# yardenas/ethz-safe-learning

Measured on AMD Instinct MI355X. Metric: planning steps/sec (CEM-MPC, N=2000 K=5 H=30), higher is better.
Workload: dtype f32

## Files before the change

ethz_safe_learning_amd/_capi.py:

```python
from __future__ import annotations

import ctypes as C
import os

CEM_ABI_VERSION = 4
CEM_MAX_ACT = 32
CEM_MAX_COST_KINDS = 4
CEM_COMM_ID_BYTES = 128
CEM_MAX_BATCH = 256
CEM_TRAIN_MAX_BATCH = 4096
CEM_INIT_COLD, CEM_INIT_EXPLICIT, CEM_INIT_SHIFT = 0, 1, 2
CEM_VARIANT_CEM, CEM_VARIANT_SAFE, CEM_VARIANT_COST = 0, 1, 2
CEM_PARTICLES_MEAN, CEM_PARTICLES_LOWER_TAIL = 0, 1
CEM_CONSTRAINT_BETA, CEM_CONSTRAINT_BUDGET = 0, 1
CEM_REFIT_UNIFORM, CEM_REFIT_SOFTMAX = 0, 1
CEM_NOISE_WHITE, CEM_NOISE_MIXED = 0, 1
CEM_FORWARD_SPLIT, CEM_FORWARD_ALL = 0, 1

_HERE = os.path.dirname(os.path.abspath(__file__))
LIB_PATH = os.environ.get('CEM_MPC_LIB') or os.path.join(_HERE, 'lib', 'libcem_mpc_gfx950.so')

EXPORTED_SYMBOLS = [
    'cem_abi_version', 'cem_status_string', 'cem_last_hip_error', 'cem_weight_blob_floats',
    'cem_packed_weight_floats', 'cem_workspace_bytes', 'cem_pack_weights_host', 'cem_plan_tiles_host', 'cem_plan_segments_host', 'cem_rollout_residency',
    'cem_planner_create', 'cem_planner_destroy', 'cem_planner_layout', 'cem_planner_set_weights', 'cem_planner_set_weights_dev',
    'cem_planner_set_normaliser', 'cem_planner_plan', 'cem_plan_begin', 'cem_plan_rollout', 'cem_plan_select',
    'cem_plan_end', 'cem_comm_unique_id', 'cem_planner_comm_init', 'cem_planner_comm_destroy', 'cem_planner_comm_ranks', 'cem_plan_exchange', 'cem_planner_graph_status', 'cem_planner_launches_per_iteration', 'cem_planner_rollout_path', 'cem_unfold_sequences', 'cem_compute_objective', 'cem_scorer_reward', 'cem_scorer_cost', 'cem_fill_noise', 'cem_philox_words', 'cem_planner_set_timing', 'cem_planner_last_timing', 'cem_planner_last_timing_detail', 'cem_planner_select_mode', 'cem_planner_inject_fault',
    'cem_batch_workspace_bytes', 'cem_batch_planner_create', 'cem_planner_plan_batch', 'cem_planner_batch_capacity',
    'cem_planner_set_warm_start', 'cem_planner_set_initial_distribution', 'cem_planner_set_init_mode', 'cem_planner_reset_carry',
    'cem_planner_get_carry', 'cem_planner_set_carry_slots', 'cem_planner_set_particle_objective', 'cem_planner_get_particle_objective',
    'cem_planner_set_constraint', 'cem_planner_get_constraint', 'cem_planner_set_cost_budget', 'cem_planner_constraint_costs',
    'cem_planner_set_refit', 'cem_planner_get_refit', 'cem_planner_refit_stats',
    'cem_planner_set_action_noise', 'cem_planner_get_action_noise', 'cem_planner_action_noise_dev',
    'cem_trainer_workspace_bytes', 'cem_trainer_blob_floats', 'cem_trainer_create', 'cem_trainer_destroy', 'cem_trainer_set_state',
    'cem_trainer_get_state', 'cem_trainer_weights_dev', 'cem_trainer_step', 'cem_trainer_steps', 'cem_trainer_eval', 'cem_trainer_forward',
]


class CemScorer(C.Structure):
    _fields_ = [
        ('goal_mode', C.c_int32), ('goal_lo', C.c_int32), ('goal_hi', C.c_int32),
        ('lidar_max_dist', C.c_float), ('goal_size', C.c_float), ('goal_reached_dist', C.c_float), ('reward_distance', C.c_float),
        ('reward_goal', C.c_float), ('reward_clip', C.c_float),
        ('constrain_indicator', C.c_int32), ('n_cost_kinds', C.c_int32),
        ('cost_lo', C.c_int32 * CEM_MAX_COST_KINDS), ('cost_hi', C.c_int32 * CEM_MAX_COST_KINDS),
        ('cost_size', C.c_float * CEM_MAX_COST_KINDS),
    ]


class CemConfig(C.Structure):
# ... 69 lines not shown
    lib.cem_planner_set_weights.argtypes = [vp, vp, C.c_size_t]
    lib.cem_planner_set_weights_dev.argtypes = [vp, vp, C.c_size_t]
    lib.cem_planner_set_normaliser.argtypes = [vp, vp, vp]
    lib.cem_planner_plan.argtypes = [vp, vp, C.c_uint64, C.c_uint64, vp, vp, vp, vp, fp, i32p]
    lib.cem_plan_begin.argtypes = [vp, vp, C.c_uint64, C.c_uint64, vp, vp]
    lib.cem_plan_rollout.argtypes = [vp, C.c_int32]
    lib.cem_plan_select.argtypes = [vp, C.c_int32]
    lib.cem_plan_end.argtypes = [vp, vp, vp, fp, i32p]
    lib.cem_unfold_sequences.argtypes = [vp, vp, vp, C.c_int32, C.c_int32, vp, C.c_uint64, C.c_uint64, vp, vp, vp]
    lib.cem_comm_unique_id.argtypes = [vp]
    lib.cem_planner_comm_init.argtypes = [vp, vp, C.c_int32, C.c_int32]
    lib.cem_planner_comm_destroy.argtypes = [vp]
    lib.cem_plan_exchange.argtypes = [vp]
    lib.cem_planner_graph_status.argtypes = [vp, i32p]
    lib.cem_planner_comm_ranks.argtypes = [vp, i32p]
    lib.cem_planner_launches_per_iteration.argtypes = [vp, i32p]
    lib.cem_planner_rollout_path.argtypes = [vp, i32p]
    lib.cem_compute_objective.argtypes = [vp, vp, C.c_int32, C.c_int32, vp]
    lib.cem_scorer_reward.argtypes = [vp, vp, vp, C.c_int32, vp, vp]
    lib.cem_scorer_cost.argtypes = [vp, vp, C.c_int32, vp]
    lib.cem_fill_noise.argtypes = [vp, C.c_uint64, C.c_uint64, vp, vp, vp]
    lib.cem_philox_words.argtypes = [vp, C.c_uint64, C.c_uint64] + [C.c_uint32] * 6 + [vp]
    lib.cem_planner_select_mode.argtypes = [vp, i32p]
    lib.cem_planner_inject_fault.argtypes = [vp, C.c_int32]
    lib.cem_planner_set_timing.argtypes = [vp, C.c_int32]
    lib.cem_planner_last_timing.argtypes = [vp, fp, i32p, fp]
    lib.cem_planner_last_timing_detail.argtypes = [vp, fp, fp]
    lib.cem_batch_workspace_bytes.restype = C.c_size_t
    lib.cem_batch_workspace_bytes.argtypes = [cfgp, C.c_int32]
    lib.cem_batch_planner_create.argtypes = [cfgp, C.c_int32, vp, C.c_size_t, vp, C.POINTER(vp)]
    lib.cem_planner_plan_batch.argtypes = [vp, C.c_int32, vp, C.c_uint64, vp, vp, vp, vp, vp, vp, vp]
    lib.cem_planner_batch_capacity.argtypes = [vp, i32p]
    lib.cem_planner_set_warm_start.argtypes = [vp, C.POINTER(CemWarmStart)]
    lib.cem_planner_set_initial_distribution.argtypes = [vp, C.c_int32, vp, vp]
    lib.cem_planner_set_init_mode.argtypes = [vp, C.c_int32, C.c_int32]
    lib.cem_planner_reset_carry.argtypes = [vp, C.c_int32]
    lib.cem_planner_get_carry.argtypes = [vp, C.c_int32, vp, vp, i32p]
    lib.cem_planner_set_carry_slots.argtypes = [vp, C.c_int32, vp]
    lib.cem_planner_set_particle_objective.argtypes = [vp, C.c_int32, C.c_int32]
    lib.cem_planner_get_particle_objective.argtypes = [vp, i32p, i32p]
    lib.cem_planner_set_constraint.argtypes = [vp, C.c_int32, C.c_int32]
    lib.cem_planner_get_constraint.argtypes = [vp, i32p, i32p]
    lib.cem_planner_set_cost_budget.argtypes = [vp, vp, C.c_int32]
    lib.cem_planner_constraint_costs.argtypes = [vp, C.c_int32, vp, C.c_int32]
    lib.cem_planner_set_refit.argtypes = [vp, C.c_int32, C.c_float]
    lib.cem_planner_get_refit.argtypes = [vp, i32p, fp]
# ... 32 lines not shown
```

ethz_safe_learning_amd/csrc/cem_capi.hip:

```cpp
#include "cem_device.h"
#include "cem_rollout_lean.h"
#include "cem_score.h"
#include "cem_refit_weighted.h"
#include "cem_noise_mix.h"
#include "cem_train.h"
#include "cem_train_tile.h"
#include "cem_forward.h"
#include "cem_rollout_split.h"
#include "cem_rollout_wide.h"
#include "cem_pack.h"
#include "../../include/cem_mpc.h"

#include <dlfcn.h>
#include <link.h>

#include <algorithm>
#include <atomic>
#include <chrono>
#include <cmath>
#include <cstdio>
#include <cstdlib>
#include <cstring>
#include <limits>
#include <mutex>
#include <new>
#include <string>
#include <type_traits>
// ... 6 lines not shown

struct Dims {
    int O, A, Din, U, L, E, P, N, H, k, I, W, R;
    int Nloc, n_off, Bloc, Btot;
    int KB_in, KB_obs, NFW, KF0;
    int act_q0, act_nq;
    bool wide;
    bool split;
    int wave_groups[4]; uint32_t wave_off_f4[4]; uint32_t member_stride_f4;
    size_t nat_member_floats;
};

int resolve_select_mode(int requested, long long N, long long k, long long HA, size_t dyn_limit, bool can_fuse, bool *cache_out)
{
    const size_t base = (size_t)((k + 3) & ~3ll) * 4 + (size_t)2 * HA * 4;
    const bool one_wg_ok = k <= 24576 && base <= dyn_limit;
    const bool cache = one_wg_ok && base + (size_t)CEM_SEL_KWORDS(N) * 4 <= dyn_limit;
    if (cache_out) *cache_out = cache;
    int mode = requested;
    if (mode == 0) mode = (N >= 24000 || !cache) ? 3 : 1;
    if (mode == 1 && !one_wg_ok) return 0;
    if (mode == 3 && !can_fuse) mode = 2;
    return mode;
}

int validate(const cem_config_t *c)
{
    if (!c) return CEM_ERR_INVALID_ARG;
    if (c->abi_version != CEM_ABI_VERSION) return CEM_ERR_INVALID_ARG;
    if (c->obs_dim < 1 || c->act_dim < 1 || c->act_dim > CEM_MAX_ACT || c->n_layers < 1 || c->ensemble_size < 1 ||
        c->particles < 1 || c->n_samples < 1 || c->horizon < 1 || c->horizon > 65535 || c->iterations < 1 || c->iterations > 65535 ||
        c->n_elite < 1 || c->n_elite > c->n_samples || c->world_size < 1 || c->rank < 0 || c->rank >= c->world_size)
        return CEM_ERR_INVALID_ARG;
    if (c->units < 1) return CEM_ERR_INVALID_ARG;
    if (c->activation < CEM_ACT_RELU || c->activation > CEM_ACT_GELU) return CEM_ERR_INVALID_ARG;
    if (!(fabs((double)c->one_minus_smoothing - (1.0 - (double)c->smoothing)) <= 2e-7)) return CEM_ERR_INVALID_ARG;
    if (c->units > CEM_WIDE_U) return CEM_ERR_UNSUPPORTED;
    if (c->obs_dim + c->act_dim > CEM_U) return CEM_ERR_UNSUPPORTED;
    if (c->n_samples % c->world_size != 0) return CEM_ERR_INVALID_ARG;
    if (((long long)c->particles * c->n_samples) % c->ensemble_size != 0) return CEM_ERR_SPLIT;
    if (c->select_mode >= 0 && c->select_mode <= 3 &&
        resolve_select_mode(c->select_mode, c->n_samples, c->n_elite, (long long)c->horizon * c->act_dim, 140 * 1024, true, nullptr) == 0)
        return CEM_ERR_UNSUPPORTED;
    if (c->scorer.n_cost_kinds < 0 || c->scorer.n_cost_kinds > CEM_MAX_COST_KINDS) return CEM_ERR_INVALID_ARG;
    {
        const cem_scorer_t &s = c->scorer;
// ... 507 lines not shown
        dl_iterate_phdr(count_hip_runtimes, &libs);
        if (libs.size() > 1) {
            std::fprintf(stderr, "cem_mpc: %zu HIP runtimes are loaded in this process:", libs.size());
            for (const auto &l : libs) std::fprintf(stderr, " %s", l.c_str());
            std::fprintf(stderr, "\ncem_mpc: device memory and streams of one are foreign to the other — load libcem_mpc_gfx950.so AFTER the runtime that owns them (INTEGRATION.md)\n");
        }
    });
}
}

struct cem_planner {
    cem_config_t cfg;
    Dims d;
    Layout lay;
    char *ws;
    hipStream_t stream;
    bool own_stream;
    int rc;
    int n_tiles;
    int n_seg, seg_len, n_pinned;
    bool have_weights;
    bool in_plan;
    bool sample_in_rollout;
    bool lean_rollout;
    const float *eps_act, *eps_model;
    CtrlBlock *h_ctrl;
    float *h_result;
    WarmCtl *h_warm; const WarmCtl *d_h_warm;
    uint32_t plan_seq;
    const CtrlBlock *d_h_ctrl; float *d_h_result;
    bool timing; std::vector<hipEvent_t> ev; float roll_ms, sel_ms, red_ms, samp_ms; int roll_n;
    std::vector<std::pair<int, int>> ev_kind;
    hipGraph_t graph; hipGraphExec_t gexec; bool graph_ready;
    ScorerDev sc;
    ScorerDev sc_roll;
    float alpha, beta;
    void *comm;
    int plans_since_comm;
    bool graph_failed;
    size_t sel_dyn_limit;
    int fused_resident;
    bool sel_zeroed;
    bool fuse_banned;
    bool inject_capture_fail;
    uint32_t inject_next;
    char *scratch; size_t scratch_bytes;
// ... 172 lines not shown
{
    int st = mb ? validate_batch(cfg, mb) : validate(cfg); if (st) return st;
    if (!workspace || !out) return CEM_ERR_INVALID_ARG;
    warn_if_two_hip_runtimes();
    cem_planner *h = new (std::nothrow) cem_planner();
    if (!h) return CEM_ERR_INVALID_ARG;
    h->cfg = *cfg; h->d = make_dims(cfg);
    h->batch = mb; h->n_states = warm_slots(h);
    const size_t nb = (size_t)warm_slots(h);
    h->lay = make_layout(cfg, h->d, max_tiles_of(h->d), mb);
    if (workspace_bytes < h->lay.total || ((uintptr_t)workspace & 255)) { delete h; return CEM_ERR_WORKSPACE; }
    h->ws = (char *)workspace; h->stream = (hipStream_t)hip_stream; h->own_stream = false;
    if (!h->stream) {
        if (hipStreamCreateWithFlags(&h->stream, hipStreamNonBlocking) != hipSuccess) { g_last_hip = (int)hipGetLastError(); delete h; return CEM_ERR_HIP; }
        h->own_stream = true;
    }
    { const Plan pl = make_plan(cfg, h->d, mb); h->rc = pl.rc; h->n_seg = pl.n_seg; h->seg_len = pl.seg_len; h->n_pinned = pl.n_pinned;
      const int slots = real_cus() * ((h->d.wide || h->d.split) ? 1 : resident_workgroups(h->d.NFW, pl.rc, pl.n_seg > 1));
      h->sample_in_rollout = (long long)nb * pl.n_tiles <= slots;
      if (const char *e = std::getenv("CEM_FORCE_SAMPLER"))
          h->sample_in_rollout = std::strcmp(e, "kernel") != 0;
      h->lean_rollout = lean_eligible(h, pl.rc);
      if (const char *e = std::getenv("CEM_FORCE_ROLLOUT"))
          h->lean_rollout = h->lean_rollout && std::strcmp(e, "generic") != 0; }
    h->have_weights = false; h->in_plan = false; h->eps_act = h->eps_model = nullptr;
    h->timing = false; h->roll_ms = h->sel_ms = h->red_ms = h->samp_ms = 0.f; h->roll_n = 0;
    h->graph = nullptr; h->gexec = nullptr; h->graph_ready = false; h->tail_m = 0;
    h->cost_m = 0; h->budget_dev = nullptr; h->cstat_obj = nullptr; h->cstat_obj_n = 0; h->last_cstat = nullptr; h->last_cstat_n = h->last_cstat_problems = 0;
    h->refit_kind = CEM_REFIT_UNIFORM; h->refit_tau = 0.f; h->refit_beta = 0.f; h->refit_dev = nullptr; h->refit_ran = false;
    h->noise_kind = CEM_NOISE_WHITE; h->noise_dev = nullptr; h->noise_eps = nullptr; h->noise_floats = 0;
    h->h_budget.assign(nb, std::numeric_limits<float>::infinity());
    h->comm = nullptr; h->plans_since_comm = 0; h->graph_failed = false;
    h->h_ctrl = nullptr; h->h_result = nullptr; h->h_warm = nullptr; h->d_h_warm = nullptr; h->pack_desc = nullptr; h->n_pack_desc = 0;
    h->warm = cem_warm_start_t{}; h->warm.shift = 1; h->warm_staged = 0; h->warm_save_skipped = false;
    h->slot_mode.assign(nb, CEM_INIT_COLD); h->carry_valid.assign(nb, 0); h->have_expl.assign(nb, 0); h->carry_at.assign(nb, -1);
    h->slot_of.resize(nb); for (size_t b = 0; b < nb; ++b) h->slot_of[b] = (int32_t)b;
    h->h_expl.assign(nb * 2 * h->d.H * h->d.A, 0.f);
    h->scratch = nullptr; h->scratch_bytes = 0; h->sel_zeroed = false; h->plan_seq = 0; h->fuse_banned = false; h->inject_next = 0; h->inject_capture_fail = false;
    auto fail = [&](int status) { g_last_hip = (int)hipGetLastError(); release_handle(h); return status; };
    const size_t result_bytes = mb ? nb * CEM_RESULT_WORDS * 4 : 64 * 4;
    if (hipHostMalloc((void **)&h->h_ctrl, nb * sizeof(CtrlBlock), hipHostMallocMapped | hipHostMallocCoherent) != hipSuccess ||
        hipHostMalloc((void **)&h->h_result, result_bytes, hipHostMallocMapped | hipHostMallocCoherent) != hipSuccess ||
        hipHostMalloc((void **)&h->h_warm, sizeof(WarmCtl) + nb * sizeof(WarmProb), hipHostMallocMapped | hipHostMallocCoherent) != hipSuccess) return fail(CEM_ERR_HIP);
    {
        const std::vector<PackDesc> table = build_pack_table(h->d);
        h->n_pack_desc = (uint32_t)table.size();
        const size_t image_bytes = h->d.wide ? wide_image_floats(h->d) * 4 : (size_t)h->d.member_stride_f4 * 16 - 4096;
// ... 482 lines not shown
        if (!h->sel_zeroed) HIPCHK(hipMemsetAsync(m.hist, 0, CEM_MS_CLEAR_BYTES, h->stream));
        h->sel_zeroed = false;
        if (mode == 3) {
            hipLaunchKernelGGL(cem_msel_fused_kernel, dim3(m.G), dim3(1024), 0, h->stream, m);
            hipLaunchKernelGGL(cem_msel_solo_kernel, dim3(1), dim3(1024), 0, h->stream, m);
        } else {
            hipLaunchKernelGGL(cem_msel_hist_kernel<0>, dim3(m.G), dim3(1024), 0, h->stream, m);
            hipLaunchKernelGGL(cem_msel_hist_kernel<1>, dim3(m.G), dim3(1024), 0, h->stream, m);
            hipLaunchKernelGGL(cem_msel_hist_kernel<2>, dim3(m.G), dim3(1024), 0, h->stream, m);
            hipLaunchKernelGGL(cem_msel_count_kernel, dim3(m.G), dim3(1024), 0, h->stream, m);
            hipLaunchKernelGGL(cem_msel_compact_kernel, dim3(m.G), dim3(1024), 0, h->stream, m);
            hipLaunchKernelGGL(cem_msel_moments_kernel<0>, dim3(m.G2), dim3(256), 0, h->stream, m);
            hipLaunchKernelGGL(cem_msel_moments_kernel<1>, dim3(m.G2), dim3(256), 0, h->stream, m);
            hipLaunchKernelGGL(cem_msel_final_kernel, dim3(1), dim3(256), 0, h->stream, m);
        }
    } else {
        if (fold_final && !h->batch && !weighted) {
            p.is_last = it == d.I - 1;
            p.result = h->d_h_result; p.result_dev = (uint32_t *)(ws + l.result); p.eps_out = have_eps_out ? (const float *)(ws + l.eps_out) : nullptr; p.noise_stddev = h->cfg.noise_stddev;
            if (folded) *folded = true;
        }
        if (cache) lds += (size_t)CEM_SEL_KWORDS(d.N) * 4;
        const dim3 grid(warm_slots(h));
        if (cache && h->cfg.variant != CEM_VARIANT_CEM) hipLaunchKernelGGL((cem_select_kernel<true, true>), grid, dim3(1024), lds, h->stream, p);
        else if (cache) hipLaunchKernelGGL((cem_select_kernel<true, false>), grid, dim3(1024), lds, h->stream, p);
        else hipLaunchKernelGGL((cem_select_kernel<false, false>), grid, dim3(1024), lds, h->stream, p);
        if (weighted) {
            HIPCHK(hipGetLastError());
            RefitWeightedParams rw{}; rw.scores = p.scores; rw.actions = p.actions; rw.musig = (float *)(ws + l.musig); rw.ctrl = p.ctrl; rw.elite_idx = p.elite_idx;
            rw.stat = h->refit_dev + (size_t)warm_slots(h) * 2 * p.HA;
            rw.N = d.N; rw.k = d.k; rw.HA = p.HA; rw.I = d.I; rw.beta = h->refit_beta;
            rw.smoothing = p.smoothing; rw.one_minus_smoothing = p.one_minus_smoothing; rw.threshold = h->cfg.stddev_threshold;
            HIPCHK(launch_refit_weighted(rw, warm_slots(h), h->stream));
            h->refit_ran = true;
        }
    }
    HIPCHK(hipGetLastError());
    return CEM_OK;
}

int enqueue_exchange(cem_planner *h)
{
    if (!h->comm) return CEM_OK;
    Rccl *r = rccl(); if (!r) return CEM_ERR_COMM;
    const Dims &d = h->d; const Layout &l = h->lay;
    NCCLCHK(r->AllGather(h->ws + l.scores_local, h->ws + l.scores_global, (size_t)d.Nloc, kNcclFloat32, h->comm, h->stream));
    return CEM_OK;
// ... 778 lines not shown
    HIPCHK(hipStreamSynchronize(h->stream));
    return CEM_OK;
}

int cem_philox_words(cem_planner_t *h, uint64_t seed, uint64_t call, uint32_t stream, uint32_t iteration, uint32_t t, uint32_t sub,
                     uint32_t idx0, uint32_t n, uint32_t *words_out_dev)
{
    if (!h || !words_out_dev || stream > 2 || iteration > 65535 || t > 65535 || sub > 65535) return CEM_ERR_INVALID_ARG;
    if (h->in_plan) return CEM_ERR_STATE;
    if (n == 0) return CEM_OK;
    int st = upload_key(h, seed, call); if (st) return st;
    WordsParams wp{}; wp.out = words_out_dev; wp.ctrl = (const CtrlBlock *)(h->ws + h->lay.ctrl);
    wp.stream = stream; wp.it = iteration; wp.t = t; wp.sub = sub; wp.idx0 = idx0; wp.n = n;
    hipLaunchKernelGGL(cem_philox_words_kernel, dim3((n + 255) / 256), dim3(256), 0, h->stream, wp);
    HIPCHK(hipGetLastError());
    HIPCHK(hipStreamSynchronize(h->stream));
    return CEM_OK;
}

int cem_planner_select_mode(const cem_planner_t *h, int32_t *mode_out)
{
    if (!h || !mode_out) return CEM_ERR_INVALID_ARG;
    *mode_out = select_mode_now(h);
    return CEM_OK;
}

int cem_planner_inject_fault(cem_planner_t *h, int32_t kind)
{
    if (!h || (kind != 1 && kind != 2)) return CEM_ERR_INVALID_ARG;
    if (h->in_plan) return CEM_ERR_STATE;
    if (kind == 2) { h->inject_capture_fail = true; return CEM_OK; }
    h->inject_next = 1u;
    return CEM_OK;
}

int cem_planner_set_timing(cem_planner_t *h, int32_t enable)
{
    if (!h) return CEM_ERR_INVALID_ARG;
    h->timing = enable != 0;
    return CEM_OK;
}

int cem_planner_last_timing(cem_planner_t *h, float *rollout_ms_total, int32_t *rollout_launches, float *select_ms_total)
{
    if (!h) return CEM_ERR_INVALID_ARG;
    if (rollout_ms_total) *rollout_ms_total = h->roll_ms;
// ... 303 lines not shown
```

ethz_safe_learning_amd/csrc/cem_device.h:

```cpp
#pragma once
#include <hip/hip_runtime.h>
#include <stdint.h>

typedef float f4 __attribute__((ext_vector_type(4)));

#define CEM_U 128
#define CEM_ET_NMIN 0
#define CEM_ET_RDELTA 1
#define CEM_ET_BMU 2
#define CEM_ET_BVAR 3
#define CEM_ET_OBS 4
#define CEM_ET_ACT 5
#define CEM_ET_SEL0 6
#define CEM_ET_SEL1 7
#define CEM_ET_ROWS 8
#define CEM_NG 8
#define CEM_NKIND 5
#define CEM_PART_FLOATS (CEM_NKIND * 4 * 64)
#define CEM_TAB_LDS_BYTES (CEM_ET_ROWS * CEM_U * 4)
#define CEM_ROLLOUT_LDS_BYTES(RC_) ((size_t)2 * (RC_) * CEM_NG * 1024 + CEM_PART_FLOATS * 4 + CEM_TAB_LDS_BYTES)

struct TileDesc {
    int32_t row_base;
    int32_t cnt;
// ... 893 lines not shown

struct ScorerOpParams {
    const float *obs, *next_obs; float *out; uint8_t *flag;
    int32_t n, O, what;
    ScorerDev sc;
};

__global__ __launch_bounds__(256) void cem_scorer_kernel(const ScorerOpParams p)
{
    const int row = (int)((blockIdx.x * 256u + threadIdx.x) >> 4), j = threadIdx.x & 15;
    if (row >= p.n) return;
    const float *o = p.obs + (size_t)row * p.O;
    if (p.what == 1) {
        const float c = cem_cost16(o, p.sc, j);
        if (j == 0) p.out[row] = c;
        return;
    }
    const float d = cem_goal_dist16(o, p.sc, j), dn = cem_goal_dist16(p.next_obs + (size_t)row * p.O, p.sc, j);
    const bool ga = d <= p.sc.goal_thresh;
    const float r = cem_reward_of(d, dn, ga, p.sc);
    if (j == 0) { p.out[row] = r; if (p.flag) p.flag[row] = ga ? 1 : 0; }
}

__device__ __forceinline__ float cem_out_noise(const CtrlBlock *ctrl, const float *eps_out, const int a)
{
    if (eps_out) return eps_out[a];
    const f4 e = cem_normal4((uint32_t)(a >> 2), 0u, 0u, 0u, CEM_STREAM_OUT, cem_key(ctrl));
    return e[a & 3];
}


#define CEM_RESULT_WORDS 38
#define CEM_RESULT_MAGIC 0x5EC0DE5Au
__host__ __device__ inline uint32_t cem_result_checksum(const volatile uint32_t *w, const uint32_t seq)
{
    uint32_t x = CEM_RESULT_MAGIC ^ seq;
    for (int i = 0; i < 36; ++i) x = (x ^ w[i]) * 0x01000193u;
    return x ^ (x >> 15);
}
__device__ __forceinline__ void cem_emit_result(float *result, uint32_t *result_dev, const uint32_t *res_l , const uint32_t seq, const int lane)
{
    const uint32_t x = cem_result_checksum(res_l, seq);
    if (lane < CEM_RESULT_WORDS) {
        const uint32_t w = lane < 36 ? res_l[lane] : (lane == 36 ? seq : x);
        if (result_dev) result_dev[lane] = w;
        __hip_atomic_store(reinterpret_cast<uint32_t *>(result) + lane, w, __ATOMIC_RELAXED, __HIP_MEMORY_SCOPE_SYSTEM);
// ... 69 lines not shown
    const int b0 = 2 * tid, b1 = 2 * tid + 1;
    uint32_t h0 = 0u, h1 = 0u;
    if (COHERENT) {
        if (b0 < nbins) h0 = __hip_atomic_load(h + b0, __ATOMIC_RELAXED, __HIP_MEMORY_SCOPE_AGENT);
        if (b1 < nbins) h1 = __hip_atomic_load(h + b1, __ATOMIC_RELAXED, __HIP_MEMORY_SCOPE_AGENT);
    } else { h0 = b0 < nbins ? h[b0] : 0u; h1 = b1 < nbins ? h[b1] : 0u; }
    const uint32_t tot = h0 + h1;
    uint32_t inc = tot;
#pragma unroll
    for (int d = 1; d < 64; d <<= 1) { const uint32_t o = __shfl_up(inc, d); if (lane >= d) inc += o; }
    if (lane == 63) sh[wv] = inc;
    __syncthreads();
    uint32_t before = 0, all = 0;
    for (int i = 0; i < 16; ++i) { const uint32_t v = sh[i]; all += v; if (i < wv) before += v; }
    const uint32_t above = all - (before + inc);
    const uint32_t ge1 = h1 + above, ge0 = tot + above;
    if (ge1 >= need && above < need) { sh[16] = (uint32_t)b1; sh[17] = need - above; }
    if (ge0 >= need && ge1 < need) { sh[16] = (uint32_t)b0; sh[17] = need - ge1; }
    __syncthreads();
    bin = sh[16]; need_next = sh[17];
    __syncthreads();
}

template <bool CACHE, bool CROWDED = false>
__global__ __launch_bounds__(1024) void cem_select_kernel(const SelectParams p)
{
    extern __shared__ __attribute__((aligned(16))) char sel_smem[];
    __shared__ __attribute__((aligned(16))) uint32_t hist[2][256];
    __shared__ uint32_t wsum[2][16];
    __shared__ uint32_t sh_prefix, sh_need, sh_cnt;
    __shared__ uint32_t sh20[20];
    __shared__ __attribute__((aligned(16))) float red[4096];
    __shared__ float bsc[16];
    __shared__ int bpos[16];
    const int prob = (int)blockIdx.x;
    CtrlBlock *const ctrl = p.ctrl + prob;
    if (p.check_done && ctrl->done) return;
    const float *const scores_b = p.scores + (size_t)prob * p.N;
    const float *const actions_b = p.actions + (size_t)prob * p.N * p.HA;
    float *const musig_b = p.musig + (size_t)prob * 2 * p.HA;
    int32_t *const elite_b = p.elite_idx + (size_t)prob * p.k;
    const float *const ret_b = p.ret ? p.ret + (size_t)prob * p.P * p.N : p.ret;
    float *const scores_wb = p.scores_w ? p.scores_w + (size_t)prob * p.N : p.scores_w;

    const int tid = threadIdx.x;
    const int N = p.N, k = p.k, HA = p.HA;
// ... 922 lines not shown
```

ethz_safe_learning_amd/planner.py:

```python
from __future__ import annotations

import ctypes as C
import math
from dataclasses import dataclass, field
from typing import List, Optional, Sequence, Tuple

import numpy as np

from . import _capi


@dataclass
class ScorerConfig:
    goal_slice: Tuple[int, int]
    observe_goal_lidar: bool = True
    lidar_max_dist: float = 4.0
    goal_size: float = 0.3
    reward_distance: float = 1.0
    reward_goal: float = 1.0
    reward_clip: float = 10.0
    constrain_indicator: bool = True
    cost_kinds: List[Tuple[int, int, float]] = field(default_factory=list)


# ... 477 lines not shown
        ptr, n = C.c_void_p(), C.c_size_t()
        _capi.check(self.lib.cem_planner_action_noise_dev(self.h, C.byref(ptr), C.byref(n)), 'cem_planner_action_noise_dev')
        per = c.iterations * c.n_samples * c.horizon * c.act_dim
        if not ptr.value:
            raise RuntimeError('the handle has no mixed action noise (set_action_noise was never given a matrix)')
        if not 0 <= int(problem) < n.value // per:
            raise ValueError('problem out of range')

        class _Dev:
            __cuda_array_interface__ = dict(shape=(per,), typestr='<f4', data=(ptr.value + 4 * per * int(problem), False), version=2)
        self.synchronize()
        with t.cuda.device(self.device):
            out = t.as_tensor(_Dev(), device=self.device).cpu().numpy().copy()
        return out.reshape(c.iterations, c.n_samples, c.horizon, c.act_dim)

    def plan_exchange(self):
        _capi.check(self.lib.cem_plan_exchange(self.h), 'cem_plan_exchange')

    def select_mode(self):
        m = C.c_int32()
        _capi.check(self.lib.cem_planner_select_mode(self.h, C.byref(m)), 'cem_planner_select_mode')
        return m.value

    def inject_fault(self, kind=1):
        _capi.check(self.lib.cem_planner_inject_fault(self.h, kind), 'cem_planner_inject_fault')

    INIT_MODES = {'cold': _capi.CEM_INIT_COLD, 'explicit': _capi.CEM_INIT_EXPLICIT, 'shift': _capi.CEM_INIT_SHIFT}

    def n_slots(self):
        return self.max_batch

    def set_warm_start(self, shift=1, tail='box', sigma='reset', floor_frac=0.0):
        tails, rules = {'box': 0, 'repeat': 1}, {'reset': 0, 'keep': 1}
        if tail not in tails or sigma not in rules:
            raise ValueError("tail is 'box' or 'repeat', sigma is 'reset' or 'keep'")
        ws = _capi.CemWarmStart(shift=int(shift), tail=tails[tail], sigma_rule=rules[sigma])
        ws.sigma_floor[:self.cfg.act_dim] = warm_sigma_floor(self.cfg, floor_frac).tolist()
        _capi.check(self.lib.cem_planner_set_warm_start(self.h, C.byref(ws)), 'cem_planner_set_warm_start')

    def set_initial_distribution(self, mu, sigma, slot=0):
        c = self.cfg
        m = np.ascontiguousarray(np.asarray(mu, np.float32))
        s = np.ascontiguousarray(np.asarray(sigma, np.float32))
        if m.shape != (c.horizon, c.act_dim) or s.shape != (c.horizon, c.act_dim):
            raise ValueError('mu and sigma must have shape [%d, %d]' % (c.horizon, c.act_dim))
        _capi.check(self.lib.cem_planner_set_initial_distribution(self.h, int(slot), _np_ptr(m), _np_ptr(s)), 'cem_planner_set_initial_distribution')
# ... 371 lines not shown
```

include/cem_mpc.h:

```cpp
#ifndef CEM_MPC_H
#define CEM_MPC_H

#include <stddef.h>
#include <stdint.h>

#ifdef __cplusplus
extern "C" {
#endif

#define CEM_ABI_VERSION 4
#define CEM_MAX_ACT 32
#define CEM_MAX_COST_KINDS 4
#define CEM_MAX_BATCH 256

enum cem_status {
    CEM_OK = 0,
    CEM_ERR_INVALID_ARG = 1,
    CEM_ERR_UNSUPPORTED = 2,
    CEM_ERR_SPLIT = 3,
    CEM_ERR_WORKSPACE = 4,
    CEM_ERR_HIP = 5,
    CEM_ERR_NO_WEIGHTS = 6,
    CEM_ERR_STATE = 7,
    CEM_ERR_COMM = 8,
// ... 91 lines not shown
int cem_planner_layout(const cem_planner_t *h, cem_layout_t *out);

int cem_planner_set_weights(cem_planner_t *h, const float *blob, size_t n_floats);
int cem_planner_set_normaliser(cem_planner_t *h, const float *inputs_min, const float *inputs_max );
int cem_planner_set_weights_dev(cem_planner_t *h, const float *blob_dev, size_t n_floats);

int cem_planner_plan(cem_planner_t *h, const float *state, uint64_t seed, uint64_t call,
                     const float *eps_act_dev, const float *eps_model_dev, const float *eps_out_host,
                     float *action_out, float *best_score_out, int32_t *iters_out);

int cem_plan_begin(cem_planner_t *h, const float *state, uint64_t seed, uint64_t call,
                   const float *eps_act_dev, const float *eps_model_dev);
int cem_plan_rollout(cem_planner_t *h, int32_t it);
int cem_plan_select(cem_planner_t *h, int32_t it);
int cem_plan_end(cem_planner_t *h, const float *eps_out_host, float *action_out, float *best_score_out, int32_t *iters_out);

#define CEM_COMM_ID_BYTES 128
int cem_comm_unique_id(void *id_out );
int cem_planner_comm_init(cem_planner_t *h, const void *id , int32_t n_ranks, int32_t rank);
int cem_planner_comm_destroy(cem_planner_t *h);
int cem_planner_comm_ranks(const cem_planner_t *h, int32_t *n_ranks_out);
int cem_plan_exchange(cem_planner_t *h);
int cem_planner_select_mode(const cem_planner_t *h, int32_t *mode_out);
int cem_planner_inject_fault(cem_planner_t *h, int32_t kind);
int cem_planner_graph_status(const cem_planner_t *h, int32_t *status_out);
int cem_planner_launches_per_iteration(const cem_planner_t *h, int32_t *launches_out);
int cem_planner_rollout_path(const cem_planner_t *h, int32_t *path_out);

int cem_unfold_sequences(cem_planner_t *h, const float *s0_dev, const float *actions_dev, int32_t n_rows, int32_t horizon,
                         const float *eps_model_dev, uint64_t seed, uint64_t call,
                         float *traj_out_dev, float *mu_out_dev, float *sd_out_dev);

int cem_compute_objective(cem_planner_t *h, const float *traj_dev, int32_t n_rows, int32_t horizon, float *scores_out_dev);

int cem_scorer_reward(cem_planner_t *h, const float *obs_dev, const float *next_obs_dev, int32_t n, float *reward_out_dev,
                      uint8_t *goal_achieved_out_dev);
int cem_scorer_cost(cem_planner_t *h, const float *obs_dev, int32_t n, float *cost_out_dev);

int cem_fill_noise(cem_planner_t *h, uint64_t seed, uint64_t call, float *eps_act_dev, float *eps_model_dev, float *eps_out_dev);

int cem_philox_words(cem_planner_t *h, uint64_t seed, uint64_t call, uint32_t stream, uint32_t iteration, uint32_t t, uint32_t sub,
                     uint32_t idx0, uint32_t n, uint32_t *words_out_dev);

int cem_planner_set_timing(cem_planner_t *h, int32_t enable);
int cem_planner_last_timing(cem_planner_t *h, float *rollout_ms_total, int32_t *rollout_launches, float *select_ms_total);
int cem_planner_last_timing_detail(cem_planner_t *h, float *reduce_ms_total, float *sampler_ms_total);
// ... 87 lines not shown
```

Baseline: 546.3.

## Add register-resident single-workgroup elite selection kernel for small populations

Adds a specialised select kernel for the plain CEM variant with uniform refit, N up to 2048 and HA up to 1024. Each thread holds up to two scores in registers and finds the top-k threshold with a radix histogram in LDS, ballot-based elite compaction and a vectorised mean/variance refit. It replaces the generic cached select kernel on the default path and is meant to cut per-iteration selection latency. It adds a separately compiled unit linked through a weak symbol, plus an env override and query APIs.

After: 547.9 (median of 6 runs). Within noise of the previous version (+0.3%).

```diff
diff --git a/ethz_safe_learning_amd/_capi.py b/ethz_safe_learning_amd/_capi.py
--- a/ethz_safe_learning_amd/_capi.py
+++ b/ethz_safe_learning_amd/_capi.py
@@ -14,6 +14,7 @@
 CEM_PARTICLES_MEAN, CEM_PARTICLES_LOWER_TAIL = 0, 1
 CEM_CONSTRAINT_BETA, CEM_CONSTRAINT_BUDGET = 0, 1
 CEM_REFIT_UNIFORM, CEM_REFIT_SOFTMAX = 0, 1
+SELECT_KERNELS = (None, 'staged', 'crowded', 'global', 'registers', 'chain', 'fused')
 CEM_NOISE_WHITE, CEM_NOISE_MIXED = 0, 1
 CEM_FORWARD_SPLIT, CEM_FORWARD_ALL = 0, 1
 
@@ -25,7 +26,7 @@
     'cem_packed_weight_floats', 'cem_workspace_bytes', 'cem_pack_weights_host', 'cem_plan_tiles_host', 'cem_plan_segments_host', 'cem_rollout_residency',
     'cem_planner_create', 'cem_planner_destroy', 'cem_planner_layout', 'cem_planner_set_weights', 'cem_planner_set_weights_dev',
     'cem_planner_set_normaliser', 'cem_planner_plan', 'cem_plan_begin', 'cem_plan_rollout', 'cem_plan_select',
-    'cem_plan_end', 'cem_comm_unique_id', 'cem_planner_comm_init', 'cem_planner_comm_destroy', 'cem_planner_comm_ranks', 'cem_plan_exchange', 'cem_planner_graph_status', 'cem_planner_launches_per_iteration', 'cem_planner_rollout_path', 'cem_unfold_sequences', 'cem_compute_objective', 'cem_scorer_reward', 'cem_scorer_cost', 'cem_fill_noise', 'cem_philox_words', 'cem_planner_set_timing', 'cem_planner_last_timing', 'cem_planner_last_timing_detail', 'cem_planner_select_mode', 'cem_planner_inject_fault',
+    'cem_plan_end', 'cem_comm_unique_id', 'cem_planner_comm_init', 'cem_planner_comm_destroy', 'cem_planner_comm_ranks', 'cem_plan_exchange', 'cem_planner_graph_status', 'cem_planner_launches_per_iteration', 'cem_planner_rollout_path', 'cem_unfold_sequences', 'cem_compute_objective', 'cem_scorer_reward', 'cem_scorer_cost', 'cem_fill_noise', 'cem_philox_words', 'cem_planner_set_timing', 'cem_planner_last_timing', 'cem_planner_last_timing_detail', 'cem_planner_select_mode', 'cem_planner_select_kernel', 'cem_select_kernel_for', 'cem_planner_inject_fault',
     'cem_batch_workspace_bytes', 'cem_batch_planner_create', 'cem_planner_plan_batch', 'cem_planner_batch_capacity',
     'cem_planner_set_warm_start', 'cem_planner_set_initial_distribution', 'cem_planner_set_init_mode', 'cem_planner_reset_carry',
     'cem_planner_get_carry', 'cem_planner_set_carry_slots', 'cem_planner_set_particle_objective', 'cem_planner_get_particle_objective',
@@ -141,6 +142,8 @@
     lib.cem_fill_noise.argtypes = [vp, C.c_uint64, C.c_uint64, vp, vp, vp]
     lib.cem_philox_words.argtypes = [vp, C.c_uint64, C.c_uint64] + [C.c_uint32] * 6 + [vp]
     lib.cem_planner_select_mode.argtypes = [vp, i32p]
+    lib.cem_planner_select_kernel.argtypes = [vp, i32p]
+    lib.cem_select_kernel_for.argtypes = [cfgp, C.c_int32, C.c_int32, i32p]
     lib.cem_planner_inject_fault.argtypes = [vp, C.c_int32]
     lib.cem_planner_set_timing.argtypes = [vp, C.c_int32]
     lib.cem_planner_last_timing.argtypes = [vp, fp, i32p, fp]
diff --git a/ethz_safe_learning_amd/csrc/cem_capi.hip b/ethz_safe_learning_amd/csrc/cem_capi.hip
--- a/ethz_safe_learning_amd/csrc/cem_capi.hip
+++ b/ethz_safe_learning_amd/csrc/cem_capi.hip
@@ -3,6 +3,7 @@
 #include "cem_score.h"
 #include "cem_refit_weighted.h"
 #include "cem_noise_mix.h"
+#include "cem_select_small.h"
 #include "cem_train.h"
 #include "cem_train_tile.h"
 #include "cem_forward.h"
@@ -55,6 +56,17 @@
     if (mode == 1 && !one_wg_ok) return 0;
     if (mode == 3 && !can_fuse) mode = 2;
     return mode;
+}
+
+int select_kernel_of(int mode, bool cache, long long N, long long HA, int variant, int refit, bool small_ok)
+{
+    if (mode == 2) return CEM_SELECT_KERNEL_CHAIN;
+    if (mode == 3) return CEM_SELECT_KERNEL_FUSED;
+    if (mode != 1) return 0;
+    if (!cache) return CEM_SELECT_KERNEL_GLOBAL;
+    if (variant != CEM_VARIANT_CEM) return CEM_SELECT_KERNEL_CROWDED;
+    if (small_ok && launch_select_small && refit == CEM_REFIT_UNIFORM && N <= CEM_SEL_SMALL_MAX_N && HA <= CEM_SEL_SMALL_MAX_HA) return CEM_SELECT_KERNEL_REGISTERS;
+    return CEM_SELECT_KERNEL_STAGED;
 }
 
 int validate(const cem_config_t *c)
@@ -608,6 +620,7 @@
     bool have_weights;
     bool in_plan;
     bool sample_in_rollout;
+    bool small_select;
     bool lean_rollout;
     const float *eps_act, *eps_model;
     CtrlBlock *h_ctrl;
@@ -826,7 +839,10 @@
           h->sample_in_rollout = std::strcmp(e, "kernel") != 0;
       h->lean_rollout = lean_eligible(h, pl.rc);
       if (const char *e = std::getenv("CEM_FORCE_ROLLOUT"))
-          h->lean_rollout = h->lean_rollout && std::strcmp(e, "generic") != 0; }
+          h->lean_rollout = h->lean_rollout && std::strcmp(e, "generic") != 0;
+      h->small_select = true;
+      if (const char *e = std::getenv("CEM_FORCE_SELECT"))
+          h->small_select = std::strcmp(e, "generic") != 0; }
     h->have_weights = false; h->in_plan = false; h->eps_act = h->eps_model = nullptr;
     h->timing = false; h->roll_ms = h->sel_ms = h->red_ms = h->samp_ms = 0.f; h->roll_n = 0;
     h->graph = nullptr; h->gexec = nullptr; h->graph_ready = false; h->tail_m = 0;
@@ -1355,7 +1371,11 @@
         }
         if (cache) lds += (size_t)CEM_SEL_KWORDS(d.N) * 4;
         const dim3 grid(warm_slots(h));
-        if (cache && h->cfg.variant != CEM_VARIANT_CEM) hipLaunchKernelGGL((cem_select_kernel<true, true>), grid, dim3(1024), lds, h->stream, p);
+        const int kern = select_kernel_of(mode, cache, d.N, p.HA, h->cfg.variant, h->refit_kind, h->small_select);
+        if (kern == CEM_SELECT_KERNEL_REGISTERS) {
+            p.stamps += 8;
+            HIPCHK(launch_select_small(p, (int)grid.x, lds - (size_t)CEM_SEL_KWORDS(d.N) * 4, h->stream));
+        } else if (kern == CEM_SELECT_KERNEL_CROWDED) hipLaunchKernelGGL((cem_select_kernel<true, true>), grid, dim3(1024), lds, h->stream, p);
         else if (cache) hipLaunchKernelGGL((cem_select_kernel<true, false>), grid, dim3(1024), lds, h->stream, p);
         else hipLaunchKernelGGL((cem_select_kernel<false, false>), grid, dim3(1024), lds, h->stream, p);
         if (weighted) {
@@ -2180,6 +2200,27 @@
 {
     if (!h || !mode_out) return CEM_ERR_INVALID_ARG;
     *mode_out = select_mode_now(h);
+    return CEM_OK;
+}
+
+int cem_planner_select_kernel(const cem_planner_t *h, int32_t *kernel_out)
+{
+    if (!h || !kernel_out) return CEM_ERR_INVALID_ARG;
+    bool cache = false;
+    const int mode = select_mode_now(h, &cache);
+    *kernel_out = select_kernel_of(mode, cache, h->d.N, (long long)h->d.H * h->d.A, h->cfg.variant, h->refit_kind, h->small_select);
+    return CEM_OK;
+}
+
+int cem_select_kernel_for(const cem_config_t *cfg, int32_t refit, int32_t force_generic, int32_t *kernel_out)
+{
+    if (!cfg || !kernel_out || (refit != CEM_REFIT_UNIFORM && refit != CEM_REFIT_SOFTMAX)) return CEM_ERR_INVALID_ARG;
+    const int st = validate(cfg); if (st) return st;
+    const long long HA = (long long)cfg->horizon * cfg->act_dim;
+    bool cache = false;
+    const int mode = resolve_select_mode(cfg->select_mode, cfg->n_samples, cfg->n_elite, HA, 140 * 1024, true, &cache);
+    if (refit == CEM_REFIT_SOFTMAX && mode != 1) return CEM_ERR_UNSUPPORTED;
+    *kernel_out = select_kernel_of(mode, cache, cfg->n_samples, HA, cfg->variant, refit, force_generic == 0);
     return CEM_OK;
 }
 
diff --git a/ethz_safe_learning_amd/csrc/cem_device.h b/ethz_safe_learning_amd/csrc/cem_device.h
--- a/ethz_safe_learning_amd/csrc/cem_device.h
+++ b/ethz_safe_learning_amd/csrc/cem_device.h
@@ -939,6 +939,7 @@
     if (j == 0) { p.out[row] = r; if (p.flag) p.flag[row] = ga ? 1 : 0; }
 }
 
+#endif
 __device__ __forceinline__ float cem_out_noise(const CtrlBlock *ctrl, const float *eps_out, const int a)
 {
     if (eps_out) return eps_out[a];
@@ -1054,6 +1055,7 @@
     __syncthreads();
 }
 
+#ifndef CEM_DEVICE_PRIMITIVES_ONLY
 template <bool CACHE, bool CROWDED = false>
 __global__ __launch_bounds__(1024) void cem_select_kernel(const SelectParams p)
 {
diff --git a/ethz_safe_learning_amd/csrc/cem_select_small.h b/ethz_safe_learning_amd/csrc/cem_select_small.h
--- /dev/null
+++ b/ethz_safe_learning_amd/csrc/cem_select_small.h
@@ -0,0 +1,355 @@
+#pragma once
+#include "cem_device.h"
+
+#define CEM_SEL_SMALL_MAX_N 2048
+#define CEM_SEL_SMALL_MAX_HA 1024
+#define CEM_SEL_SMALL_SWZ(b) ((((b) & 28u) << 6) | (((b) >> 5) << 2) | ((b) & 3u))
+
+__attribute__((weak)) hipError_t launch_select_small(const SelectParams &p, int n_problems, size_t dyn_lds, hipStream_t st);
+
+#ifdef CEM_SELECT_SMALL_UNIT
+__global__ __launch_bounds__(1024) void cem_select_small_kernel(const SelectParams p)
+{
+    extern __shared__ __attribute__((aligned(16))) char sel_smem[];
+    __shared__ __attribute__((aligned(16))) uint32_t h2k[2048];
+    __shared__ uint32_t lkey[256], lidx[256];
+    __shared__ uint32_t wmm[2][16];
+    __shared__ uint32_t wcnt[2][16];
+    __shared__ uint32_t sh_cnt, sh_bucket, sh_need1, sh_m, sh_T, sh_need;
+    __shared__ __attribute__((aligned(16))) float red[2][4096];
+    __shared__ float bsc[16];
+    __shared__ int bpos[16];
+    __shared__ uint32_t res_l[40];
+    const int prob = (int)blockIdx.x;
+    CtrlBlock *const ctrl = p.ctrl + prob;
+    if (p.check_done && ctrl->done) return;
+    const float *const scores_b = p.scores + (size_t)prob * p.N;
+    const float *const actions_b = p.actions + (size_t)prob * p.N * p.HA;
+    float *const musig_b = p.musig + (size_t)prob * 2 * p.HA;
+    int32_t *const elite_b = p.elite_idx + (size_t)prob * p.k;
+    const float *const ret_b = p.ret ? p.ret + (size_t)prob * p.P * p.N : p.ret;
+    float *const scores_wb = p.scores_w ? p.scores_w + (size_t)prob * p.N : p.scores_w;
+
+    const int tid = threadIdx.x, lane = tid & 63, wv = tid >> 6;
+    const int N = p.N, k = p.k, HA = p.HA;
+    CEM_SEL_STAMP(0);
+    int32_t *elite = reinterpret_cast<int32_t *>(sel_smem);
+    float *newsig = reinterpret_cast<float *>(sel_smem + (size_t)((k + 3) & ~3) * 4) + HA;
+
+    float old_mu = 0.f, old_sg = 0.f;
+    if (tid < HA) { old_mu = musig_b[tid]; old_sg = musig_b[HA + tid]; }
+    float best0 = 0.f; int iters0 = 0; uint32_t seq0 = 0u;
+    if (tid == 64) best0 = ctrl->best_score;
+    if (tid == 0) iters0 = ctrl->iters;
+    if (tid < 64 && p.result) seq0 = ctrl->seq;
+
+    const int C = N > 1024 ? 2 : 1;
+    const int beg = tid * C;
+    const bool have[2] = {beg < N, C == 2 && beg + 1 < N};
+    uint32_t key[2] = {0u, 0u};
+    {
+        float v[2] = {0.f, 0.f};
+        if (ret_b) {
+            float acc[2] = {0.f, 0.f};
+            for (int q0 = 0; q0 < p.P; q0 += 8) {
+                float r[8][2];
+#pragma unroll
+                for (int j = 0; j < 2; ++j)
+                    if (j < C) {
+                        const int i = beg + j, ic = i < N ? i : N - 1;
+#pragma unroll
+                        for (int u = 0; u < 8; ++u) r[u][j] = ret_b[(size_t)(q0 + u < p.P ? q0 + u : p.P - 1) * N + ic];
+                    }
+#pragma unroll
+                for (int u = 0; u < 8; ++u)
+                    if (q0 + u < p.P) {
+#pragma unroll
+                        for (int j = 0; j < 2; ++j) if (j < C) acc[j] = acc[j] + r[u][j];
+                    }
+            }
+#pragma unroll
+            for (int j = 0; j < 2; ++j) { v[j] = acc[j] / (float)p.P; if (have[j]) scores_wb[beg + j] = v[j]; }
+        } else {
+#pragma unroll
+            for (int j = 0; j < 2; ++j) if (have[j]) v[j] = scores_b[beg + j];
+        }
+#pragma unroll
+        for (int j = 0; j < 2; ++j) key[j] = cem_f2key(v[j]);
+    }
+    uint32_t kmin = 0xFFFFFFFFu, kmax = 0u;
+#pragma unroll
+    for (int j = 0; j < 2; ++j) if (have[j]) { kmin = key[j] < kmin ? key[j] : kmin; kmax = key[j] > kmax ? key[j] : kmax; }
+#pragma unroll
+    for (int d = 32; d >= 1; d >>= 1) {
+        const uint32_t a = (uint32_t)__shfl_xor((int)kmin, d), b = (uint32_t)__shfl_xor((int)kmax, d);
+        kmin = a < kmin ? a : kmin; kmax = b > kmax ? b : kmax;
+    }
+    if (lane == 0) { wmm[0][wv] = kmin; wmm[1][wv] = kmax; }
+    h2k[tid] = 0u; h2k[tid + 1024] = 0u;
+    if (tid == 0) sh_cnt = 0u;
+    if (tid < 40) res_l[tid] = 0u;
+    __syncthreads();
+    for (int i = 0; i < 16; ++i) { kmin = wmm[0][i] < kmin ? wmm[0][i] : kmin; kmax = wmm[1][i] > kmax ? wmm[1][i] : kmax; }
+    CEM_SEL_STAMP(1);
+
+    uint32_t T = 0u, need = (uint32_t)k;
+    {
+        uint32_t base = kmin, window = kmax - kmin;
+        int sh = window ? max(0, 21 - (int)__clz((int)window)) : 0;
+#pragma unroll 1
+        for (int level = 0; level < 4; ++level) {
+#pragma unroll
+            for (int j = 0; j < 2; ++j) {
+                const uint32_t off = key[j] - base;
+                if (have[j] && off <= window) atomicAdd(&h2k[CEM_SEL_SMALL_SWZ(off >> sh)], 1u);
+            }
+            __syncthreads();
+            if (wv == 0) {
+                uint4 h[8];
+#pragma unroll
+                for (int q = 0; q < 8; ++q) h[q] = *reinterpret_cast<const uint4 *>(&h2k[256 * q + 4 * lane]);
+                uint32_t tot = 0u;
+#pragma unroll
+                for (int q = 0; q < 8; ++q) tot += h[q].x + h[q].y + h[q].z + h[q].w;
+                uint32_t suf = tot;
+#pragma unroll
+                for (int d = 1; d < 64; d <<= 1) { const uint32_t o = __shfl_down(suf, d); if (lane + d < 64) suf += o; }
+                const uint64_t straddles = __builtin_amdgcn_ballot_w64(suf - tot < need && suf >= need);
+                const int L = straddles ? __builtin_ctzll(straddles) : 0;
+                const uint32_t above = (uint32_t)__shfl((int)(suf - tot), L);
+                const uint32_t c = lane < 32 ? h2k[CEM_SEL_SMALL_SWZ((uint32_t)(32 * L + lane))] : 0u;
+                uint32_t s2 = c;
+#pragma unroll
+                for (int d = 1; d < 32; d <<= 1) { const uint32_t o = __shfl_down(s2, d); if (lane + d < 64) s2 += o; }
+                const uint32_t run = above + s2 - c;
+                if (run < need && run + c >= need) { sh_bucket = (uint32_t)(32 * L + lane); sh_need1 = need - run; sh_m = c; }
+            }
+            __syncthreads();
+            const uint32_t bucket = sh_bucket, need1 = sh_need1, m = sh_m;
+            if (sh == 0) { T = base + bucket; need = need1; break; }
+            if (m <= 256u) {
+#pragma unroll
+                for (int j = 0; j < 2; ++j) {
+                    const uint32_t off = key[j] - base;
+                    if (have[j] && off <= window && (off >> sh) == bucket) { const uint32_t pos = atomicAdd(&sh_cnt, 1u); if (pos < 256u) { lkey[pos] = key[j]; lidx[pos] = (uint32_t)(beg + j); } }
+                }
+                __syncthreads();
+                if ((uint32_t)tid < m) {
+                    const uint32_t kj = lkey[tid], ij = lidx[tid];
+                    uint32_t gt = 0, before = 0;
+                    for (uint32_t l = 0; l < m; ++l) { const uint32_t kl = lkey[l]; gt += kl > kj; before += (kl > kj) || (kl == kj && lidx[l] < ij); }
+                    if (before == need1 - 1u) { sh_T = kj; sh_need = need1 - gt; }
+                }
+                __syncthreads();
+                T = sh_T; need = sh_need;
+                break;
+            }
+            base += bucket << sh; window = (1u << sh) - 1u; need = need1;
+            sh = sh > 11 ? sh - 11 : 0;
+            __syncthreads();
+            h2k[tid] = 0u; h2k[tid + 1024] = 0u;
+            __syncthreads();
+        }
+    }
+    CEM_SEL_STAMP(2);
+
+    {
+        const bool g0 = have[0] && key[0] > T, g1 = have[1] && key[1] > T, e0 = have[0] && key[0] == T, e1 = have[1] && key[1] == T;
+        const uint64_t bg0 = __builtin_amdgcn_ballot_w64(g0), bg1 = __builtin_amdgcn_ballot_w64(g1);
+        const uint64_t be0 = __builtin_amdgcn_ballot_w64(e0), be1 = __builtin_amdgcn_ballot_w64(e1);
+        const uint64_t below = (1ull << lane) - 1ull;
+        uint32_t pre_gt = (uint32_t)(__builtin_popcountll(bg0 & below) + __builtin_popcountll(bg1 & below));
+        uint32_t pre_eq = (uint32_t)(__builtin_popcountll(be0 & below) + __builtin_popcountll(be1 & below));
+        if (lane == 0) {
+            wcnt[0][wv] = (uint32_t)(__builtin_popcountll(bg0) + __builtin_popcountll(bg1));
+            wcnt[1][wv] = (uint32_t)(__builtin_popcountll(be0) + __builtin_popcountll(be1));
+        }
+        __syncthreads();
+        for (int i = 0; i < 16; ++i) if (i < wv) { pre_gt += wcnt[0][i]; pre_eq += wcnt[1][i]; }
+        uint32_t eqr = pre_eq;
+        uint32_t pos = pre_gt + (pre_eq < need ? pre_eq : need);
+        float bs = -__builtin_inff(); int bp = 0x7fffffff;
+#pragma unroll
+        for (int j = 0; j < 2; ++j)
+            if (have[j]) {
+                const int i = beg + j;
+                bool take = key[j] > T;
+                if (key[j] == T) { take = eqr < need; ++eqr; }
+                if (take && pos < (uint32_t)k) {
+                    elite[pos] = i; elite_b[pos] = i; ++pos;
+                    const float sc = cem_key2f(key[j]);
+                    if (bp == 0x7fffffff || sc > bs) { bs = sc; bp = i; }
+                }
+            }
+#pragma unroll
+        for (int d = 32; d >= 1; d >>= 1) {
+            const float os = __shfl_xor(bs, d); const int op = __shfl_xor(bp, d);
+            if (op != 0x7fffffff && (bp == 0x7fffffff || os > bs || (os == bs && op < bp))) { bs = os; bp = op; }
+        }
+        if (lane == 0) { bsc[wv] = bs; bpos[wv] = bp; }
+    }
+    __syncthreads();
+    CEM_SEL_STAMP(3);
+    float tbs = 0.f; int tbp = 0x7fffffff; bool better = false; float pre[4] = {0.f, 0.f, 0.f, 0.f};
+    if (tid == 64) {
+        tbs = bsc[0]; tbp = bpos[0];
+        for (int i = 1; i < 16; ++i) {
+            const float os = bsc[i]; const int op = bpos[i];
+            if (op != 0x7fffffff && (tbp == 0x7fffffff || os > tbs || (os == tbs && op < tbp))) { tbs = os; tbp = op; }
+        }
+        better = tbs > best0;
+#pragma unroll
+        for (int r = 0; r < 4; ++r) if (r < p.A) pre[r] = better ? actions_b[(size_t)tbp * HA + r] : ctrl->best[r];
+    }
+    CEM_SEL_STAMP(4);
+
+    const float fk = (float)k;
+    const float sm = p.smoothing, osm = p.one_minus_smoothing;
+    {
+        int tpc1 = 1; while (tpc1 * 2 * HA <= 1024) tpc1 *= 2;
+        if ((HA & 3) == 0 && k > 16 * tpc1) {
+            const int ncol4 = HA >> 2;
+            int tpc = 1; while (tpc * 2 * ncol4 <= 1024) tpc *= 2;
+            const int part = tid / ncol4, c4 = tid % ncol4;
+            const bool act = part < tpc;
+            f4 *red4a = reinterpret_cast<f4 *>(red[0]), *red4b = reinterpret_cast<f4 *>(red[1]);
+            const f4 *act4 = reinterpret_cast<const f4 *>(actions_b);
+            const f4 zero4 = (f4){0.f, 0.f, 0.f, 0.f};
+            f4 av[8];
+#pragma unroll
+            for (int j = 0; j < 8; ++j) {
+                const int e = part + j * tpc;
+                av[j] = (act && e < k) ? act4[(size_t)elite[e] * ncol4 + c4] : zero4;
+            }
+            f4 mean4 = zero4;
+            for (int phase = 0; phase < 2; ++phase) {
+                f4 acc = zero4;
+                if (act) {
+#pragma unroll
+                    for (int j = 0; j < 8; ++j)
+                        if (part + j * tpc < k) { const f4 a = av[j]; acc = phase ? acc + (a - mean4) * (a - mean4) : acc + a; }
+                    for (int e0 = part + 8 * tpc; e0 < k; e0 += 8 * tpc) {
+                        f4 b[8];
+#pragma unroll
+                        for (int j = 0; j < 8; ++j) { const int e = e0 + j * tpc; b[j] = e < k ? act4[(size_t)elite[e] * ncol4 + c4] : zero4; }
+#pragma unroll
+                        for (int j = 0; j < 8; ++j)
+                            if (e0 + j * tpc < k) { const f4 a = b[j]; acc = phase ? acc + (a - mean4) * (a - mean4) : acc + a; }
+                    }
+                }
+                f4 *const r4 = phase ? red4b : red4a;
+                r4[tid] = acc;
+                __syncthreads();
+                if (act && (!phase || part == 0)) {
+                    f4 tot = zero4;
+                    for (int pp = 0; pp < tpc; ++pp) tot = tot + r4[pp * ncol4 + c4];
+                    if (!phase) {
+#pragma unroll
+                        for (int r = 0; r < 4; ++r) mean4[r] = tot[r] / fk;
+                    } else {
+#pragma unroll
+                        for (int r = 0; r < 4; ++r) {
+                            const float sd = sqrtf(tot[r] / fk);
+                            const int ci = 4 * c4 + r;
+                            const float nsg = sm * musig_b[HA + ci] + osm * sd;
+                            musig_b[ci] = sm * musig_b[ci] + osm * mean4[r];
+                            musig_b[HA + ci] = nsg;
+                            newsig[ci] = nsg;
+                        }
+                    }
+                }
+            }
+        } else {
+            const int ncol = HA;
+            int tpc = 1; while (tpc * 2 * ncol <= 1024) tpc *= 2;
+            const int part = tid / ncol, col = tid % ncol;
+            const bool act = part < tpc;
+            float av[16];
+#pragma unroll
+            for (int j = 0; j < 16; ++j) {
+                const int e = part + j * tpc;
+                av[j] = (act && e < k) ? actions_b[(size_t)elite[e] * HA + col] : 0.f;
+            }
+            float m = 0.f;
+            for (int phase = 0; phase < 2; ++phase) {
+                float acc = 0.f;
+                if (act) {
+#pragma unroll
+                    for (int j = 0; j < 16; ++j) {
+                        const int e = part + j * tpc;
+                        if (e < k) { const float a = av[j]; acc = phase ? acc + (a - m) * (a - m) : acc + a; }
+                    }
+                    for (int e0 = part + 16 * tpc; e0 < k; e0 += 8 * tpc) {
+                        float b[8];
+#pragma unroll
+                        for (int j = 0; j < 8; ++j) { const int e = e0 + j * tpc; b[j] = e < k ? actions_b[(size_t)elite[e] * HA + col] : 0.f; }
+#pragma unroll
+                        for (int j = 0; j < 8; ++j)
+                            if (e0 + j * tpc < k) { const float a = b[j]; acc = phase ? acc + (a - m) * (a - m) : acc + a; }
+                    }
+                }
+                float *const r1 = red[phase];
+                r1[tid] = acc;
+                __syncthreads();
+                if (act && (!phase || part == 0)) {
+                    float tot = 0.f;
+                    for (int pp = 0; pp < tpc; ++pp) tot = tot + r1[pp * ncol + col];
+                    if (!phase) m = tot / fk;
+                    else {
+                        const float sd = sqrtf(tot / fk);
+                        const float nsg = sm * old_sg + osm * sd;
+                        musig_b[col] = sm * old_mu + osm * m;
+                        musig_b[HA + col] = nsg;
+                        newsig[col] = nsg;
+                    }
+                }
+            }
+        }
+    }
+    __syncthreads();
+    CEM_SEL_STAMP(5);
+    if (tid == 0) {
+        float ssum = 0.f;
+        for (int i = 0; i < HA; ++i) ssum = ssum + newsig[i];
+        const float mean_sigma = ssum / (float)HA;
+        const int iters = iters0 + 1;
+        const bool stop = mean_sigma <= p.threshold;
+        ctrl->iters = iters;
+        if (stop) ctrl->done = 1;
+        if (p.result) {
+            res_l[33] = (uint32_t)iters; res_l[34] = stop ? 1u : (uint32_t)ctrl->done; res_l[35] = (uint32_t)ctrl->fault;
+            res_l[36] = (stop || p.is_last != 0) ? 1u : 0u;
+        }
+        CEM_SEL_STAMP(6);
+    }
+    if (tid == 64) {
+        const float bs = tbs;
+        const int idx = tbp;
+        for (int a0 = 0; a0 < p.A; a0 += 4) {
+            f4 e = (f4){0.f, 0.f, 0.f, 0.f};
+            if (p.result && !p.eps_out) e = cem_normal4((uint32_t)(a0 >> 2), 0u, 0u, 0u, CEM_STREAM_OUT, cem_key(ctrl));
+#pragma unroll
+            for (int r = 0; r < 4; ++r) {
+                const int a = a0 + r;
+                if (a < p.A) {
+                    const float b = a0 == 0 ? pre[r] : (better ? actions_b[(size_t)idx * HA + a] : ctrl->best[a]);
+                    if (better) ctrl->best[a] = b;
+                    if (p.result) res_l[a] = __float_as_uint(b + (p.eps_out ? p.eps_out[a] : e[r]) * p.noise_stddev);
+                }
+            }
+        }
+        if (better) ctrl->best_score = bs;
+        if (p.result) res_l[32] = __float_as_uint(better ? bs : best0);
+    }
+    if (p.result) {
+        __syncthreads();
+        if (tid < 64 && res_l[36]) cem_emit_result(p.result, p.result_dev, res_l, seq0, tid);
+    }
+}
+
+hipError_t launch_select_small(const SelectParams &p, int n_problems, size_t dyn_lds, hipStream_t st)
+{
+    hipLaunchKernelGGL(cem_select_small_kernel, dim3(n_problems), dim3(1024), dyn_lds, st, p);
+    return hipGetLastError();
+}
+#endif
diff --git a/ethz_safe_learning_amd/csrc/cem_select_small.hip b/ethz_safe_learning_amd/csrc/cem_select_small.hip
--- /dev/null
+++ b/ethz_safe_learning_amd/csrc/cem_select_small.hip
@@ -0,0 +1,3 @@
+#define CEM_DEVICE_PRIMITIVES_ONLY
+#define CEM_SELECT_SMALL_UNIT
+#include "cem_select_small.h"
diff --git a/ethz_safe_learning_amd/planner.py b/ethz_safe_learning_amd/planner.py
--- a/ethz_safe_learning_amd/planner.py
+++ b/ethz_safe_learning_amd/planner.py
@@ -523,6 +523,11 @@
         _capi.check(self.lib.cem_planner_select_mode(self.h, C.byref(m)), 'cem_planner_select_mode')
         return m.value
 
+    def select_kernel(self):
+        m = C.c_int32()
+        _capi.check(self.lib.cem_planner_select_kernel(self.h, C.byref(m)), 'cem_planner_select_kernel')
+        return _capi.SELECT_KERNELS[m.value]
+
     def inject_fault(self, kind=1):
         _capi.check(self.lib.cem_planner_inject_fault(self.h, kind), 'cem_planner_inject_fault')
 
diff --git a/include/cem_mpc.h b/include/cem_mpc.h
--- a/include/cem_mpc.h
+++ b/include/cem_mpc.h
@@ -137,6 +137,10 @@
 int cem_planner_comm_ranks(const cem_planner_t *h, int32_t *n_ranks_out);
 int cem_plan_exchange(cem_planner_t *h);
 int cem_planner_select_mode(const cem_planner_t *h, int32_t *mode_out);
+enum cem_select_kernel { CEM_SELECT_KERNEL_STAGED = 1, CEM_SELECT_KERNEL_CROWDED = 2, CEM_SELECT_KERNEL_GLOBAL = 3, CEM_SELECT_KERNEL_REGISTERS = 4,
+                         CEM_SELECT_KERNEL_CHAIN = 5, CEM_SELECT_KERNEL_FUSED = 6 };
+int cem_planner_select_kernel(const cem_planner_t *h, int32_t *kernel_out);
+int cem_select_kernel_for(const cem_config_t *cfg, int32_t refit, int32_t force_generic, int32_t *kernel_out);
 int cem_planner_inject_fault(cem_planner_t *h, int32_t kind);
 int cem_planner_graph_status(const cem_planner_t *h, int32_t *status_out);
 int cem_planner_launches_per_iteration(const cem_planner_t *h, int32_t *launches_out);
```
